# marja-w/gan-des-midi-music-gen

Hardware: AMD Instinct MI355X
Metric: GAN training samples/sec (G+D step) (higher is better)
Workload: dtype bf16; 1 GPU; SIMNN G/D iteration, synthetic 128x256 spectrogram windows; per_gpu_batch=256, global_batch=256, mode=faithful, parallelism=dp1

## Files before the change

gan_des_midi_music_gen_amd/csrc/adam_pc.h:

```cpp
#pragma once
#include "gdm_common.h"

__device__ __forceinline__ void adam_derived(const float* hyper, int step, float& step_size, float& bc2_sqrt) {
  const double b1 = (double)hyper[2], b2 = (double)hyper[3];
  step_size = (float)((double)hyper[1] / (1.0 - pow(b1, (double)step)));
  bc2_sqrt = (float)sqrt(1.0 - pow(b2, (double)step));
}

__device__ __forceinline__ void adam_pc_gather(float (&tile)[32][132], const float* __restrict__ g_pc, int C, int P,
                                               int bx, int by, int bz) {
  const int t = threadIdx.x, tx = t & 31, ty = t >> 5;
  const int p0 = bx * 128, c0 = by * 32;
  const int64_t base = (int64_t)bz * C * P;
#pragma unroll
  for (int i = 0; i < 16; ++i) {
    const int pl = ty + 8 * i, pp = p0 + pl, c = c0 + tx;
    tile[tx][pl] = (pp < P && c < C) ? g_pc[base + (int64_t)pp * C + c] : 0.f;
  }
}

template <typename TS>
__device__ __forceinline__ void adam_pc_update(float (&tile)[32][132], float* __restrict__ p, float* __restrict__ m,
                                               float* __restrict__ v, int C, int P, TS* __restrict__ shadow_pc,
                                               const float* __restrict__ hyper, int vec_ok, float step_size,
                                               float bc2_sqrt, int bx, int by, int bz) {
  const float w1 = 1.0f - hyper[2], beta2 = hyper[3], omb2 = 1.0f - hyper[3], eps = hyper[4], gscale = hyper[5];
  const int t = threadIdx.x, tx = t & 31, ty = t >> 5;
  const int p0 = bx * 128, c0 = by * 32, n = bz;
  const int64_t base = (int64_t)n * C * P;
  const bool full = vec_ok && p0 + 128 <= P && c0 + 32 <= C;
#pragma unroll
  for (int i = 0; i < 4; ++i) {
    const int cl = ty + 8 * i, c = c0 + cl, pp = p0 + 4 * tx;
    const int64_t k = base + (int64_t)c * P + pp;
    f32x4 gg = *(const f32x4*)&tile[cl][4 * tx], pv, mv, vv;
    if (full) {
#ifndef GDM_ADAM_DEFAULT_POLICY
      pv = __builtin_nontemporal_load((const f32x4*)(p + k)); mv = __builtin_nontemporal_load((const f32x4*)(m + k));
      vv = __builtin_nontemporal_load((const f32x4*)(v + k));
#else
      pv = *(const f32x4*)(p + k); mv = *(const f32x4*)(m + k); vv = *(const f32x4*)(v + k);
#endif
    } else {
#pragma unroll
      for (int e = 0; e < 4; ++e) {
        const bool ok = c < C && pp + e < P;
        pv[e] = ok ? p[k + e] : 0.f; mv[e] = ok ? m[k + e] : 0.f; vv[e] = ok ? v[k + e] : 0.f;
      }
    }
#pragma unroll
    for (int e = 0; e < 4; ++e) {
      float pj = pv[e], mj = mv[e], vj = vv[e];
      adam_element(pj, mj, vj, gg[e], gscale, w1, beta2, omb2, eps, step_size, bc2_sqrt);
      pv[e] = pj; mv[e] = mj; vv[e] = vj;
    }
    if (full) {
#ifndef GDM_ADAM_DEFAULT_POLICY
      __builtin_nontemporal_store(pv, (f32x4*)(p + k)); __builtin_nontemporal_store(mv, (f32x4*)(m + k));
      __builtin_nontemporal_store(vv, (f32x4*)(v + k));
#else
      *(f32x4*)(p + k) = pv; *(f32x4*)(m + k) = mv; *(f32x4*)(v + k) = vv;
#endif
    } else {
#pragma unroll
      for (int e = 0; e < 4; ++e)
        if (c < C && pp + e < P) { p[k + e] = pv[e]; m[k + e] = mv[e]; v[k + e] = vv[e]; }
    }
    *(f32x4*)&tile[cl][4 * tx] = pv;
  }
  __syncthreads();
#pragma unroll
  for (int i = 0; i < 16; ++i) {
    const int pl = ty + 8 * i, pp = p0 + pl, c = c0 + tx;
    if (pp < P && c < C) shadow_pc[base + (int64_t)pp * C + c] = from_f32<TS>(tile[tx][pl]);
  }
}


template <typename TS>
__device__ __forceinline__ void adam_pc_tile(float (&tile)[32][132], float* __restrict__ p, const float* __restrict__ g_pc,
                                             float* __restrict__ m, float* __restrict__ v, int C, int P,
                                             TS* __restrict__ shadow_pc, const float* __restrict__ hyper, int vec_ok,
                                             float step_size, float bc2_sqrt, int bx, int by, int bz) {
  adam_pc_gather(tile, g_pc, C, P, bx, by, bz);
  __syncthreads();
  adam_pc_update<TS>(tile, p, m, v, C, P, shadow_pc, hyper, vec_ok, step_size, bc2_sqrt, bx, by, bz);
}
```

gan_des_midi_music_gen_amd/csrc/pointwise.hip:

```cpp
#include "gdm_common.h"
#include "adam_pc.h"

namespace {

__global__ __launch_bounds__(1024) void bce_kernel(const float* __restrict__ x, float target, int n, float gscale,
                                                   float* __restrict__ loss, float* __restrict__ dx, int fuse_sig,
                                                   int accumulate) {
  __shared__ float red[1024];
  const int t = threadIdx.x;
  float s = 0.f;
  for (int i = t; i < n; i += 1024) {
    const float v = x[i];
    s += fmaxf(v, 0.f) - v * target + log1pf(expf(-fabsf(v)));
    if (dx) {
      float g = (1.0f / (1.0f + expf(-v)) - target) * gscale / (float)n;
      if (fuse_sig) g *= v * (1.f - v);
      dx[i] = g;
    }
  }
  red[t] = s;
  __syncthreads();
  for (int o = 512; o > 0; o >>= 1) {
    if (t < o) red[t] += red[t + o];
    __syncthreads();
// ... 85 lines not shown
        pp[j] = pj; mm[j] = mj; vv[j] = vj;
      }
      *(f32x4*)(p + i) = pp;
      *(f32x4*)(m + i) = mm;
      *(f32x4*)(v + i) = vv;
    } else {
      for (int64_t k = i; k < n && k < i + 4; ++k) {
        adam_element(p[k], m[k], v[k], g[k], gscale, w1, beta2, omb2, eps, step_size, bc2_sqrt);
      }
    }
  }
}

struct Welford { float n, mean, m2; };
__device__ __forceinline__ void welford_merge(Welford& a, const Welford& b) {
  if (b.n == 0.f) return;
  const float n = a.n + b.n;
  const float d = b.mean - a.mean;
  a.mean += d * (b.n / n);
  a.m2 += b.m2 + d * d * (a.n * b.n / n);
  a.n = n;
}

__device__ __forceinline__ Welford welford_from_shifted(float n, float shift, float s, float ss) {
  Welford a{n, 0.f, 0.f};
  if (n > 0.f) {
    a.mean = shift + s / n;
    a.m2 = fmaxf(ss - s * (s / n), 0.f);
  }
  return a;
}

__global__ __launch_bounds__(256) void bn_partial_stats(const float* __restrict__ y, int rows, int C, int chunk_rows,
                                                        int CW, float* __restrict__ ws) {
  __shared__ Welford sh[4][64];
  const int lane = threadIdx.x & 63, wv = threadIdx.x >> 6;
  const int rpl = 64 / CW;
  const int c = blockIdx.x * 64 + (lane & (CW - 1)), sub = lane / CW;
  const int r0 = blockIdx.y * chunk_rows, r1 = min(rows, r0 + chunk_rows);
  const int step = 4 * rpl;
  float n = 0.f, shift = 0.f, s = 0.f, ss = 0.f;
  if (c < C) {
    int r = r0 + wv * rpl + sub;
    if (r < r1) shift = y[(int64_t)r * C + c];
    for (; r + 7 * step < r1; r += 8 * step) {
      float x[8];
#pragma unroll
      for (int q = 0; q < 8; ++q) x[q] = y[(int64_t)(r + q * step) * C + c];
#pragma unroll
      for (int q = 0; q < 8; ++q) { const float d = x[q] - shift; s += d; ss += d * d; }
      n += 8.f;
    }
    for (; r < r1; r += step) { const float d = y[(int64_t)r * C + c] - shift; s += d; ss += d * d; n += 1.f; }
  }
  sh[wv][lane] = welford_from_shifted(n, shift, s, ss);
  __syncthreads();
  if (wv == 0 && sub == 0 && c < C) {
    Welford t{0.f, 0.f, 0.f};
    for (int w = 0; w < 4; ++w)
      for (int q = 0; q < rpl; ++q) welford_merge(t, sh[w][q * CW + lane]);
    float* o = ws + ((int64_t)blockIdx.y * C + c) * 3;
    o[0] = t.n; o[1] = t.mean; o[2] = t.m2;
  }
}

__global__ __launch_bounds__(1024) void bn_finalize(const float* __restrict__ ws, int chunks, int rows, int C,
                                                    float momentum, float eps, float* __restrict__ running_mean,
                                                    float* __restrict__ running_var, int64_t* __restrict__ nbt,
                                                    float* __restrict__ save_mean, float* __restrict__ save_invstd) {
  __shared__ Welford part[16][64];
  const int lane = threadIdx.x & 63, wv = threadIdx.x >> 6;
  const int c = blockIdx.x * 64 + lane;
  if (blockIdx.x == 0 && threadIdx.x == 0 && nbt) nbt[0] += 1;
  Welford t{0.f, 0.f, 0.f};
  if (c < C)
    for (int k = wv; k < chunks; k += 16 * 8) {
      Welford b[8];
#pragma unroll
      for (int q = 0; q < 8; ++q) {
        const int kk = k + 16 * q;
        const float* o = ws + ((int64_t)min(kk, chunks - 1) * C + c) * 3;
        b[q] = Welford{kk < chunks ? o[0] : 0.f, o[1], o[2]};
      }
#pragma unroll
      for (int q = 0; q < 8; ++q) welford_merge(t, b[q]);
    }
  part[wv][lane] = t;
  __syncthreads();
  if (wv != 0 || c >= C) return;
  t = part[0][lane];
#pragma unroll
  for (int w = 1; w < 16; ++w) welford_merge(t, part[w][lane]);
  const float var_b = t.m2 / (float)rows;
  save_mean[c] = t.mean;
  save_invstd[c] = 1.0f / sqrtf(var_b + eps);
  if (running_mean) {
    const float var_u = t.m2 / (float)max(rows - 1, 1);
    running_mean[c] = (1.f - momentum) * running_mean[c] + momentum * t.mean;
    running_var[c] = (1.f - momentum) * running_var[c] + momentum * var_u;
  }
}

__global__ __launch_bounds__(256) void bn_eval_stats(const float* __restrict__ running_mean,
                                                     const float* __restrict__ running_var, int C, float eps,
                                                     float* __restrict__ save_mean, float* __restrict__ save_invstd) {
  const int c = blockIdx.x * 256 + threadIdx.x;
  if (c >= C) return;
  save_mean[c] = running_mean[c];
  save_invstd[c] = 1.0f / sqrtf(running_var[c] + eps);
}

template <typename IT>
__global__ __launch_bounds__(256) void bn_apply(const float* __restrict__ y, int64_t total64, int C,
                                                const float* __restrict__ gamma, const float* __restrict__ beta,
                                                const float* __restrict__ mean, const float* __restrict__ invstd,
                                                int act, void* __restrict__ out, int out_dtype) {
  const IT total = (IT)total64, stride = (IT)gridDim.x * 256;
  for (IT i = (IT)blockIdx.x * 256 + threadIdx.x; i < total; i += stride) {
    const int c = (int)(i % C);
    const float alpha = invstd[c] * gamma[c];
    const float v = (y[i] - mean[c]) * alpha + beta[c];
    store_from_f32(out, out_dtype, i, apply_act(v, act, 0.f));
  }
}

__global__ __launch_bounds__(256) void bn_bwd_partial(const void* __restrict__ dout, const void* __restrict__ out,
                                                      int dtype, const float* __restrict__ y, int rows, int C,
                                                      int chunk_rows, const float* __restrict__ mean,
                                                      const float* __restrict__ invstd, int act,
                                                      float* __restrict__ ws) {
  __shared__ float sh1[4][64], sh2[4][64];
  const int lane = threadIdx.x & 63, wv = threadIdx.x >> 6;
  const int c = blockIdx.x * 64 + lane;
  const int r0 = blockIdx.y * chunk_rows, r1 = min(rows, r0 + chunk_rows);
  float s1 = 0.f, s2 = 0.f;
  if (c < C) {
    const float mu = mean[c], is = invstd[c];
    for (int r = r0 + wv; r < r1; r += 4) {
      const int64_t i = (int64_t)r * C + c;
      const float g = load_as_f32(dout, dtype, i) * act_grad_from_out(load_as_f32(out, dtype, i), act, 0.f);
      s1 += g;
      s2 += g * ((y[i] - mu) * is);
    }
  }
  sh1[wv][lane] = s1; sh2[wv][lane] = s2;
  __syncthreads();
  if (wv == 0 && c < C) {
    float* o = ws + ((int64_t)blockIdx.y * C + c) * 2;
    o[0] = ((sh1[0][lane] + sh1[1][lane]) + sh1[2][lane]) + sh1[3][lane];
    o[1] = ((sh2[0][lane] + sh2[1][lane]) + sh2[2][lane]) + sh2[3][lane];
  }
}

__global__ __launch_bounds__(256) void bn_bwd_finalize(const float* __restrict__ ws, int chunks, int C,
                                                       float* __restrict__ dgamma, float* __restrict__ dbeta) {
  const int c = blockIdx.x * 256 + threadIdx.x;
  if (c >= C) return;
  float s1 = 0.f, s2 = 0.f;
  for (int k = 0; k < chunks; ++k) {
    s1 += ws[((int64_t)k * C + c) * 2];
    s2 += ws[((int64_t)k * C + c) * 2 + 1];
  }
  dbeta[c] = s1;
  dgamma[c] = s2;
}

__global__ __launch_bounds__(256) void bn_bwd_apply(const void* __restrict__ dout, const void* __restrict__ out,
                                                    int dtype, const float* __restrict__ y, int64_t total, int rows,
                                                    int C, const float* __restrict__ gamma,
                                                    const float* __restrict__ mean, const float* __restrict__ invstd,
                                                    const float* __restrict__ dgamma, const float* __restrict__ dbeta,
                                                    int act, float* __restrict__ dy) {
  const int64_t stride = (int64_t)gridDim.x * 256;
  const float inv_r = 1.0f / (float)rows;
  for (int64_t i = (int64_t)blockIdx.x * 256 + threadIdx.x; i < total; i += stride) {
    const int c = (int)(i % C);
    const float g = load_as_f32(dout, dtype, i) * act_grad_from_out(load_as_f32(out, dtype, i), act, 0.f);
    const float xhat = (y[i] - mean[c]) * invstd[c];
    dy[i] = gamma[c] * invstd[c] * (g - dbeta[c] * inv_r - xhat * dgamma[c] * inv_r);
  }
}

__global__ __launch_bounds__(256) void bias_act_kernel(const float* __restrict__ x, const float* __restrict__ bias,
                                                       int64_t total, int cols, int act, float slope,
                                                       void* __restrict__ out, int out_dtype) {
  const int64_t stride = (int64_t)gridDim.x * 256;
  for (int64_t i = (int64_t)blockIdx.x * 256 + threadIdx.x; i < total; i += stride) {
    float v = x[i];
    if (bias) v += bias[i % cols];
    store_from_f32(out, out_dtype, i, apply_act(v, act, slope));
  }
}

__global__ __launch_bounds__(256) void act_bwd_kernel(const void* __restrict__ dout, const void* __restrict__ out,
                                                      int dtype, int64_t n, int act, float slope,
                                                      void* __restrict__ dx) {
  const int64_t stride = (int64_t)gridDim.x * 256;
  for (int64_t i = (int64_t)blockIdx.x * 256 + threadIdx.x; i < n; i += stride) {
    const float g = load_as_f32(dout, dtype, i) * act_grad_from_out(load_as_f32(out, dtype, i), act, slope);
    store_from_f32(dx, dtype, i, g);
  }
}

__global__ __launch_bounds__(256) void colsum_partial(const void* __restrict__ x, int dtype, int rows, int C,
                                                      int chunk_rows, float* __restrict__ ws) {
  __shared__ float sh[4][64];
  const int lane = threadIdx.x & 63, wv = threadIdx.x >> 6;
  const int c = blockIdx.x * 64 + lane;
  const int r0 = blockIdx.y * chunk_rows, r1 = min(rows, r0 + chunk_rows);
  float s = 0.f;
  if (c < C)
    for (int r = r0 + wv; r < r1; r += 4) s += load_as_f32(x, dtype, (int64_t)r * C + c);
  sh[wv][lane] = s;
  __syncthreads();
  if (wv == 0 && c < C) ws[(int64_t)blockIdx.y * C + c] = ((sh[0][lane] + sh[1][lane]) + sh[2][lane]) + sh[3][lane];
}

__global__ __launch_bounds__(256) void colsum_final(const float* __restrict__ ws, int chunks, int C,
                                                    float* __restrict__ out) {
  const int c = blockIdx.x * 256 + threadIdx.x;
  if (c >= C) return;
  float s = 0.f;
  for (int k = 0; k < chunks; ++k) s += ws[(int64_t)k * C + c];
  out[c] = s;
}

__global__ __launch_bounds__(256) void cast_kernel(const void* __restrict__ src, int sd, void* __restrict__ dst,
                                                   int dd, int64_t n) {
  const int64_t stride = (int64_t)gridDim.x * 256;
  for (int64_t i = (int64_t)blockIdx.x * 256 + threadIdx.x; i < n; i += stride)
    store_from_f32(dst, dd, i, load_as_f32(src, sd, i));
}

inline int row_chunks(int rows) {
  int c = (rows + 255) / 256;
  return c < 1 ? 1 : (c > 64 ? 64 : c);
}
inline unsigned grid_for(int64_t total) {
  int64_t b = (total + 255) / 256;
  return (unsigned)(b > 4096 ? 4096 : (b < 1 ? 1 : b));
}

}

extern "C" int gdm_bce_with_logits(const float* x, float target, int n, float grad_scale, float* loss, float* dx,
                                   int fuse_sigmoid_backward, int accumulate_loss, void* stream) {
  GDM_REQUIRE(x && loss, "gdm_bce_with_logits: null pointer");
  GDM_REQUIRE(n > 0 && n <= 65536, "gdm_bce_with_logits: n=%d out of range (1..65536)", n);
  hipLaunchKernelGGL(bce_kernel, dim3(1), dim3(1024), 0, (hipStream_t)stream, x, target, n, grad_scale, loss, dx,
                     fuse_sigmoid_backward, accumulate_loss);
  GDM_LAUNCH_OK("gdm_bce_with_logits");
  return GDM_OK;
}

extern "C" int gdm_criterion_loss(const float* x, float target, int n, int criterion, float grad_scale, float* loss,
                                  float* dx, int accumulate_loss, void* stream) {
  GDM_REQUIRE(x && loss, "gdm_criterion_loss: null pointer");
  GDM_REQUIRE(n > 0 && n <= 65536, "gdm_criterion_loss: n=%d out of range (1..65536)", n);
  GDM_REQUIRE(criterion == GDM_CRIT_BCE_LOGITS || criterion == GDM_CRIT_MSE || criterion == GDM_CRIT_L1,
              "gdm_criterion_loss: unknown criterion %d (GDM_CRIT_BCE_LOGITS, GDM_CRIT_MSE or GDM_CRIT_L1)", criterion);
  hipStream_t s = (hipStream_t)stream;
  if (criterion == GDM_CRIT_BCE_LOGITS)
    hipLaunchKernelGGL(bce_kernel, dim3(1), dim3(1024), 0, s, x, target, n, grad_scale, loss, dx, 0, accumulate_loss);
  else if (criterion == GDM_CRIT_MSE)
    hipLaunchKernelGGL(crit_kernel<GDM_CRIT_MSE>, dim3(1), dim3(1024), 0, s, x, target, n, grad_scale, loss, dx,
                       accumulate_loss);
  else
    hipLaunchKernelGGL(crit_kernel<GDM_CRIT_L1>, dim3(1), dim3(1024), 0, s, x, target, n, grad_scale, loss, dx,
                       accumulate_loss);
  GDM_LAUNCH_OK("gdm_criterion_loss");
  return GDM_OK;
}

extern "C" int gdm_adam_step(float* p, const float* g, float* m, float* v, int64_t n, int step, float lr, float beta1,
                             float beta2, float eps, float grad_scale, void* stream) {
  GDM_REQUIRE(p && g && m && v, "gdm_adam_step: null pointer");
  GDM_REQUIRE(n > 0 && step >= 1, "gdm_adam_step: bad n=%lld or step=%d", (long long)n, step);
  const bool aligned = (((uintptr_t)p | (uintptr_t)g | (uintptr_t)m | (uintptr_t)v) & 15) == 0;
  const double bc1 = 1.0 - pow((double)beta1, (double)step);
  const double bc2 = 1.0 - pow((double)beta2, (double)step);
  const float step_size = (float)((double)lr / bc1);
  const float bc2_sqrt = (float)sqrt(bc2);
  int64_t blocks = (n / 4 + 255) / 256;
  if (blocks < 1) blocks = 1;
  if (blocks > 8192) blocks = 8192;
  if (aligned)
    hipLaunchKernelGGL(adam_kernel<true>, dim3((unsigned)blocks), dim3(256), 0, (hipStream_t)stream, p, g, m, v, n,
                       1.0f - beta1, beta2, 1.0f - beta2, step_size, bc2_sqrt, eps, grad_scale);
  else
    hipLaunchKernelGGL(adam_kernel<false>, dim3((unsigned)blocks), dim3(256), 0, (hipStream_t)stream, p, g, m, v, n,
                       1.0f - beta1, beta2, 1.0f - beta2, step_size, bc2_sqrt, eps, grad_scale);
  GDM_LAUNCH_OK("gdm_adam_step");
  return GDM_OK;
}

extern "C" int gdm_adam_step_dev_pc(float* p, const float* g_pc, float* m, float* v, int N, int C, int P,
                                    void* shadow_pc, int shadow_dtype, float* hyper, int advance_step, void* stream) {
  GDM_REQUIRE(p && g_pc && m && v && shadow_pc && hyper, "gdm_adam_step_dev_pc: null pointer");
  GDM_REQUIRE(N > 0 && C > 0 && P > 0 && N <= 65535 && (C + 31) / 32 <= 65535 && gdm_dtype_ok(shadow_dtype),
              "gdm_adam_step_dev_pc: bad arguments");
  hipStream_t s = (hipStream_t)stream;
  if (advance_step) hipLaunchKernelGGL(adam_prep_kernel, dim3(1), dim3(1), 0, s, hyper);
  const dim3 grid((P + 127) / 128, (C + 31) / 32, N);
  const int vec_ok = (P % 4 == 0) && ((((uintptr_t)p | (uintptr_t)m | (uintptr_t)v) & 15) == 0);
  if (shadow_dtype == GDM_BF16)
    hipLaunchKernelGGL(adam_dev_pc_kernel<__bf16>, grid, dim3(256), 0, s, p, g_pc, m, v, C, P, (__bf16*)shadow_pc, hyper,
                       vec_ok);
  else
    hipLaunchKernelGGL(adam_dev_pc_kernel<float>, grid, dim3(256), 0, s, p, g_pc, m, v, C, P, (float*)shadow_pc, hyper,
                       vec_ok);
  GDM_LAUNCH_OK("gdm_adam_step_dev_pc");
  return GDM_OK;
}

extern "C" int gdm_adam_step_dev(float* p, const float* g, float* m, float* v, int64_t n, float* hyper, void* stream) {
  GDM_REQUIRE(p && g && m && v && hyper && n > 0, "gdm_adam_step_dev: bad arguments");
  const bool aligned = (((uintptr_t)p | (uintptr_t)g | (uintptr_t)m | (uintptr_t)v) & 15) == 0;
  int64_t blocks = (n / 4 + 255) / 256;
  if (blocks < 1) blocks = 1;
  if (blocks > 8192) blocks = 8192;
  hipStream_t s = (hipStream_t)stream;
  hipLaunchKernelGGL(adam_prep_kernel, dim3(1), dim3(1), 0, s, hyper);
  if (aligned) hipLaunchKernelGGL(adam_dev_kernel<true>, dim3((unsigned)blocks), dim3(256), 0, s, p, g, m, v, n, hyper);
  else hipLaunchKernelGGL(adam_dev_kernel<false>, dim3((unsigned)blocks), dim3(256), 0, s, p, g, m, v, n, hyper);
  GDM_LAUNCH_OK("gdm_adam_step_dev");
  return GDM_OK;
}

extern "C" size_t gdm_bn_workspace_bytes(int rows, int channels) {
  return (size_t)row_chunks(rows) * (size_t)channels * 3 * sizeof(float);
}

extern "C" int gdm_bn_act_fwd(const float* y, int rows, int channels, const float* gamma, const float* beta,
                              float* running_mean, float* running_var, int64_t* num_batches_tracked, float momentum,
                              float eps, int act, void* out, int out_dtype, float* save_mean, float* save_invstd,
                              int training, void* workspace, size_t workspace_bytes, void* stream) {
  GDM_REQUIRE(y && gamma && beta && out && save_mean && save_invstd, "gdm_bn_act_fwd: null pointer");
  GDM_REQUIRE(rows > 0 && channels > 0 && gdm_dtype_ok(out_dtype), "gdm_bn_act_fwd: bad arguments");
  hipStream_t s = (hipStream_t)stream;
  const int C = channels;
  if (training) {
    GDM_REQUIRE(rows > 1, "gdm_bn_act_fwd: training-mode batch norm needs more than 1 value per channel");
    const int chunks = row_chunks(rows);
    if (!workspace || workspace_bytes < gdm_bn_workspace_bytes(rows, C)) {
      gdm_set_error("gdm_bn_act_fwd: workspace too small");
      return GDM_EWORKSPACE;
    }
    const int chunk_rows = (rows + chunks - 1) / chunks;
    int cw = 64;
    while (cw / 2 >= C && cw > 1) cw /= 2;
    hipLaunchKernelGGL(bn_partial_stats, dim3((C + 63) / 64, chunks), dim3(256), 0, s, y, rows, C, chunk_rows, cw,
                       (float*)workspace);
    hipLaunchKernelGGL(bn_finalize, dim3((C + 63) / 64), dim3(1024), 0, s, (const float*)workspace, chunks, rows, C,
                       momentum, eps, running_mean, running_var, num_batches_tracked, save_mean, save_invstd);
  } else {
    GDM_REQUIRE(running_mean && running_var, "gdm_bn_act_fwd: eval mode needs running statistics");
    hipLaunchKernelGGL(bn_eval_stats, dim3((C + 255) / 256), dim3(256), 0, s, running_mean, running_var, C, eps,
                       save_mean, save_invstd);
  }
  const int64_t total = (int64_t)rows * C;
  if (total < ((int64_t)1 << 31))
    hipLaunchKernelGGL(bn_apply<int>, dim3(grid_for(total)), dim3(256), 0, s, y, total, C, gamma, beta, save_mean,
                       save_invstd, act, out, out_dtype);
  else
    hipLaunchKernelGGL(bn_apply<int64_t>, dim3(grid_for(total)), dim3(256), 0, s, y, total, C, gamma, beta, save_mean,
                       save_invstd, act, out, out_dtype);
  GDM_LAUNCH_OK("gdm_bn_act_fwd");
  return GDM_OK;
}

extern "C" int gdm_bn_partial_chunks(int rows) { return row_chunks(rows); }

extern "C" int gdm_bn_partials(const float* y, int rows, int channels, float* partials, void* stream) {
  GDM_REQUIRE(y && partials && rows > 0 && channels > 0, "gdm_bn_partials: bad arguments");
  const int C = channels, chunks = row_chunks(rows), chunk_rows = (rows + chunks - 1) / chunks;
  int cw = 64;
  while (cw / 2 >= C && cw > 1) cw /= 2;
  hipLaunchKernelGGL(bn_partial_stats, dim3((C + 63) / 64, chunks), dim3(256), 0, (hipStream_t)stream, y, rows, C,
                     chunk_rows, cw, partials);
  GDM_LAUNCH_OK("gdm_bn_partials");
  return GDM_OK;
}

extern "C" int gdm_bn_apply(const float* y, int rows, int channels, const float* gamma, const float* beta,
                            const float* mean, const float* invstd, int act, void* out, int out_dtype, void* stream) {
  GDM_REQUIRE(y && gamma && beta && mean && invstd && out && rows > 0 && channels > 0 && gdm_dtype_ok(out_dtype),
              "gdm_bn_apply: bad arguments");
  const int64_t total = (int64_t)rows * channels;
  hipStream_t s = (hipStream_t)stream;
  if (total < ((int64_t)1 << 31))
    hipLaunchKernelGGL(bn_apply<int>, dim3(grid_for(total)), dim3(256), 0, s, y, total, channels, gamma, beta, mean, invstd,
                       act, out, out_dtype);
  else
    hipLaunchKernelGGL(bn_apply<int64_t>, dim3(grid_for(total)), dim3(256), 0, s, y, total, channels, gamma, beta, mean,
                       invstd, act, out, out_dtype);
  GDM_LAUNCH_OK("gdm_bn_apply");
  return GDM_OK;
}

extern "C" int gdm_bn_finalize(const float* ws, int chunks, int rows, int channels, float momentum, float eps,
                               float* running_mean, float* running_var, int64_t* num_batches_tracked, float* save_mean,
                               float* save_invstd, void* stream) {
  GDM_REQUIRE(ws && save_mean && save_invstd && chunks > 0 && rows > 1 && channels > 0, "gdm_bn_finalize: bad arguments");
  hipLaunchKernelGGL(bn_finalize, dim3((channels + 63) / 64), dim3(1024), 0, (hipStream_t)stream, ws, chunks, rows,
                     channels, momentum, eps, running_mean, running_var, num_batches_tracked, save_mean, save_invstd);
  GDM_LAUNCH_OK("gdm_bn_finalize");
  return GDM_OK;
}

extern "C" int gdm_bn_stats(const float* y, int rows, int channels, float* running_mean, float* running_var,
                            int64_t* num_batches_tracked, float momentum, float eps, float* save_mean,
                            float* save_invstd, void* workspace, size_t workspace_bytes, void* stream) {
  GDM_REQUIRE(y && save_mean && save_invstd && rows > 1 && channels > 0, "gdm_bn_stats: bad arguments");
  if (!workspace || workspace_bytes < gdm_bn_workspace_bytes(rows, channels)) {
    gdm_set_error("gdm_bn_stats: workspace too small");
    return GDM_EWORKSPACE;
  }
  hipStream_t s = (hipStream_t)stream;
  const int C = channels, chunks = row_chunks(rows), chunk_rows = (rows + chunks - 1) / chunks;
  int cw = 64;
  while (cw / 2 >= C && cw > 1) cw /= 2;
  hipLaunchKernelGGL(bn_partial_stats, dim3((C + 63) / 64, chunks), dim3(256), 0, s, y, rows, C, chunk_rows, cw,
                     (float*)workspace);
  hipLaunchKernelGGL(bn_finalize, dim3((C + 63) / 64), dim3(1024), 0, s, (const float*)workspace, chunks, rows, C,
                     momentum, eps, running_mean, running_var, num_batches_tracked, save_mean, save_invstd);
  GDM_LAUNCH_OK("gdm_bn_stats");
  return GDM_OK;
}

extern "C" int gdm_bn_act_bwd(const void* dout, const void* out, int out_dtype, const float* y, int rows, int channels,
                              const float* gamma, const float* save_mean, const float* save_invstd, int act,
                              float* dy, float* dgamma, float* dbeta, void* workspace, size_t workspace_bytes,
                              void* stream) {
  GDM_REQUIRE(dout && out && y && gamma && save_mean && save_invstd && dy && dgamma && dbeta,
              "gdm_bn_act_bwd: null pointer");
  GDM_REQUIRE(rows > 0 && channels > 0 && gdm_dtype_ok(out_dtype), "gdm_bn_act_bwd: bad arguments");
  const int C = channels, chunks = row_chunks(rows);
  if (!workspace || workspace_bytes < gdm_bn_workspace_bytes(rows, C)) {
    gdm_set_error("gdm_bn_act_bwd: workspace too small");
    return GDM_EWORKSPACE;
  }
  hipStream_t s = (hipStream_t)stream;
  const int chunk_rows = (rows + chunks - 1) / chunks;
  hipLaunchKernelGGL(bn_bwd_partial, dim3((C + 63) / 64, chunks), dim3(256), 0, s, dout, out, out_dtype, y, rows, C,
                     chunk_rows, save_mean, save_invstd, act, (float*)workspace);
  hipLaunchKernelGGL(bn_bwd_finalize, dim3((C + 255) / 256), dim3(256), 0, s, (const float*)workspace, chunks, C,
                     dgamma, dbeta);
  const int64_t total = (int64_t)rows * C;
  hipLaunchKernelGGL(bn_bwd_apply, dim3(grid_for(total)), dim3(256), 0, s, dout, out, out_dtype, y, total, rows, C,
                     gamma, save_mean, save_invstd, dgamma, dbeta, act, dy);
  GDM_LAUNCH_OK("gdm_bn_act_bwd");
  return GDM_OK;
}

extern "C" int gdm_bias_act_fwd(const float* x, const float* bias, int rows, int cols, int act, float slope, void* out,
                                int out_dtype, void* stream) {
  GDM_REQUIRE(x && out && rows > 0 && cols > 0 && gdm_dtype_ok(out_dtype), "gdm_bias_act_fwd: bad arguments");
  const int64_t total = (int64_t)rows * cols;
  hipLaunchKernelGGL(bias_act_kernel, dim3(grid_for(total)), dim3(256), 0, (hipStream_t)stream, x, bias, total, cols,
                     act, slope, out, out_dtype);
  GDM_LAUNCH_OK("gdm_bias_act_fwd");
  return GDM_OK;
}

extern "C" int gdm_act_bwd(const void* dout, const void* out, int dtype, int64_t n, int act, float slope, void* dx,
                           void* stream) {
  GDM_REQUIRE(dout && out && dx && n > 0 && gdm_dtype_ok(dtype), "gdm_act_bwd: bad arguments");
  hipLaunchKernelGGL(act_bwd_kernel, dim3(grid_for(n)), dim3(256), 0, (hipStream_t)stream, dout, out, dtype, n, act,
                     slope, dx);
  GDM_LAUNCH_OK("gdm_act_bwd");
  return GDM_OK;
}

extern "C" int gdm_colsum(const void* x, int dtype, int rows, int cols, float* out, void* workspace,
                          size_t workspace_bytes, void* stream) {
  GDM_REQUIRE(x && out && rows > 0 && cols > 0 && gdm_dtype_ok(dtype), "gdm_colsum: bad arguments");
  const int chunks = row_chunks(rows);
  if (!workspace || workspace_bytes < (size_t)chunks * cols * sizeof(float)) {
    gdm_set_error("gdm_colsum: workspace too small (need %zu)", (size_t)chunks * cols * sizeof(float));
    return GDM_EWORKSPACE;
  }
  hipStream_t s = (hipStream_t)stream;
  const int chunk_rows = (rows + chunks - 1) / chunks;
  hipLaunchKernelGGL(colsum_partial, dim3((cols + 63) / 64, chunks), dim3(256), 0, s, x, dtype, rows, cols, chunk_rows,
                     (float*)workspace);
  hipLaunchKernelGGL(colsum_final, dim3((cols + 255) / 256), dim3(256), 0, s, (const float*)workspace, chunks, cols,
                     out);
  GDM_LAUNCH_OK("gdm_colsum");
  return GDM_OK;
}

extern "C" int gdm_cast(const void* src, int src_dtype, void* dst, int dst_dtype, int64_t n, void* stream) {
  GDM_REQUIRE(src && dst && n > 0 && gdm_dtype_ok(src_dtype) && gdm_dtype_ok(dst_dtype), "gdm_cast: bad arguments");
  hipLaunchKernelGGL(cast_kernel, dim3(grid_for(n)), dim3(256), 0, (hipStream_t)stream, src, src_dtype, dst,
                     dst_dtype, n);
  GDM_LAUNCH_OK("gdm_cast");
  return GDM_OK;
}

namespace {
constexpr int HEAD_ROWS = 8;
__global__ __launch_bounds__(256) void simnn_head_kernel(const float* __restrict__ h1, const float* __restrict__ w2,
                                                         const float* __restrict__ b2, int n, int n0, float y0,
                                                         float y1, float* __restrict__ prob, void* __restrict__ dh1,
                                                         int dh1_bf16, float* __restrict__ partials) {
  __shared__ float dz_s[HEAD_ROWS], lt_s[HEAD_ROWS], part[2][256];
  const int t = threadIdx.x, lane = t & 63, wv = t >> 6;
  const int r0 = blockIdx.x * HEAD_ROWS, r1 = min(n, r0 + HEAD_ROWS);
  const float wa = w2[lane], wb = w2[lane + 64], bias = b2[0];
  float hv[HEAD_ROWS / 4][2];
#pragma unroll
  for (int k = 0; k < HEAD_ROWS / 4; ++k) {
    const int b = r0 + wv + 4 * k;
    hv[k][0] = b < r1 ? h1[(int64_t)b * 128 + lane] : 0.f;
    hv[k][1] = b < r1 ? h1[(int64_t)b * 128 + 64 + lane] : 0.f;
  }
#pragma unroll
  for (int k = 0; k < HEAD_ROWS / 4; ++k) {
    const int b = r0 + wv + 4 * k, bl = wv + 4 * k;
    const float s = wave_sum(hv[k][0] * wa + hv[k][1] * wb);
    if (lane == 0) {
      float lt = 0.f, dz = 0.f;
      if (b < r1) {
        const float z = s + bias;
        const float p = 1.0f / (1.0f + expf(-z));
        const bool first = b < n0;
        const float y = first ? y0 : y1;
        const float cnt = (float)(first ? n0 : n - n0);
        prob[b] = p;
        lt = (fmaxf(p, 0.f) - p * y + log1pf(expf(-fabsf(p)))) / cnt;
        dz = (1.0f / (1.0f + expf(-p)) - y) / cnt * p * (1.f - p);
      }
      lt_s[bl] = lt;
      dz_s[bl] = dz;
    }
  }
  __syncthreads();
  float* po = partials + (int64_t)blockIdx.x * 258;
  if (t == 0) {
    float l = 0.f, sdz = 0.f;
#pragma unroll
    for (int b = 0; b < HEAD_ROWS; ++b) { l += lt_s[b]; sdz += dz_s[b]; }
    po[256] = sdz;
    po[257] = l;
  }
  const int j = t & 127, grp = t >> 7;
  const float wj = w2[j];
  float s_w = 0.f, s_b1 = 0.f;
  float hh[HEAD_ROWS / 2];
#pragma unroll
  for (int k = 0; k < HEAD_ROWS / 2; ++k) {
    const int b = r0 + grp + 2 * k;
    hh[k] = b < r1 ? h1[(int64_t)b * 128 + j] : 0.f;
  }
#pragma unroll
  for (int k = 0; k < HEAD_ROWS / 2; ++k) {
    const int b = r0 + grp + 2 * k;
    const float d = dz_s[grp + 2 * k];
    const float g = hh[k] > 0.f ? d * wj : 0.f;
    if (dh1 != nullptr && b < r1) {
      if (dh1_bf16) ((__bf16*)dh1)[(int64_t)b * 128 + j] = (__bf16)g;
      else ((float*)dh1)[(int64_t)b * 128 + j] = g;
    }
    s_w = fmaf(d, hh[k], s_w);
    s_b1 += g;
  }
  part[0][t] = s_w;
  part[1][t] = s_b1;
  __syncthreads();
  if (t < 128) {
    po[t] = part[0][t] + part[0][128 + t];
    po[128 + t] = part[1][t] + part[1][128 + t];
  }
}

__global__ __launch_bounds__(320) void simnn_head_final(const float* __restrict__ partials, int groups,
                                                        float* __restrict__ loss, int accumulate_loss,
                                                        float* __restrict__ dw2, float* __restrict__ db2,
                                                        float* __restrict__ db1) {
  const int t = threadIdx.x;
  if (t >= 258) return;
  float p8[8] = {0.f, 0.f, 0.f, 0.f, 0.f, 0.f, 0.f, 0.f};
  int g = 0;
  for (; g + 8 <= groups; g += 8) {
#pragma unroll
    for (int q = 0; q < 8; ++q) p8[q] += partials[(int64_t)(g + q) * 258 + t];
  }
  for (; g < groups; ++g) p8[0] += partials[(int64_t)g * 258 + t];
  const float s = ((p8[0] + p8[1]) + (p8[2] + p8[3])) + ((p8[4] + p8[5]) + (p8[6] + p8[7]));
  if (t == 257) loss[0] = (accumulate_loss ? loss[0] : 0.f) + s;
  else if (dw2 != nullptr) {
    if (t < 128) dw2[t] = s;
    else if (t < 256) db1[t - 128] = s;
    else db2[0] = s;
  }
}
}

extern "C" size_t gdm_simnn_head_workspace_bytes(int n) {
  return (size_t)((n + HEAD_ROWS - 1) / HEAD_ROWS) * 258 * sizeof(float);
}

extern "C" int gdm_simnn_head(const float* h1, const float* w2, const float* b2, int n, int n0, float y0, float y1,
                              float* prob, float* loss, int accumulate_loss, void* dh1, int dh1_dtype, float* dw2,
                              float* db2, float* db1, void* workspace, size_t workspace_bytes, void* stream) {
  GDM_REQUIRE(h1 && w2 && b2 && prob && loss, "gdm_simnn_head: null pointer");
  GDM_REQUIRE(n > 0 && n <= 65536 && n0 > 0 && n0 <= n, "gdm_simnn_head: bad batch n=%d n0=%d", n, n0);
// ... 72 lines not shown
```

gan_des_midi_music_gen_amd/csrc/simnn_adam.hip:

```cpp
#include "simnn_trunk.h"
#include "adam_pc.h"

namespace {

constexpr int REC_SLOT0 = 16, REC_GROUP0 = 32, REC_GROUPS = 64;
constexpr int REC_INTS = REC_GROUP0 + 16 * REC_GROUPS;
template <typename T>
__global__ __launch_bounds__(256, 8) void simnn_adam_kernel(float* __restrict__ p, const float* __restrict__ g_pc,
                                                         float* __restrict__ m, float* __restrict__ v, int C, int P,
                                                         T* __restrict__ shadow_pc, int vec_ok, int tiles_x, int tiles_y,
                                                         int small_vec_ok, float* __restrict__ ps,
                                                         const float* __restrict__ gs, float* __restrict__ ms,
                                                         float* __restrict__ vs, int n_small,
                                                         const float* __restrict__ w2, T* __restrict__ wf,
                                                         T* __restrict__ wb, float* __restrict__ hyper, int* rec) {
  __shared__ __attribute__((aligned(16))) float lds[4608];
  static_assert(sizeof(lds) >= sizeof(float[32][132]), "tile");
  float (&tile)[32][132] = *reinterpret_cast<float (*)[32][132]>(lds);
  __shared__ float hy[2];
  STAMP_DECL;
  const int step = __float_as_int(hyper[0]) + 1;
  const int tag0 = rec[REC_SLOT0], tag1 = rec[REC_SLOT0 + 4];
  const float ss0 = __int_as_float(rec[REC_SLOT0 + 1]), bq0 = __int_as_float(rec[REC_SLOT0 + 2]);
  const float ss1 = __int_as_float(rec[REC_SLOT0 + 5]), bq1 = __int_as_float(rec[REC_SLOT0 + 6]);
  float step_size, bc2_sqrt;
  auto resolve = [&]() {
    const bool odd = step & 1;
    step_size = odd ? ss1 : ss0;
    bc2_sqrt = odd ? bq1 : bq0;
    if ((odd ? tag1 : tag0) != step) {
      if (threadIdx.x == 0) adam_derived(hyper, step, hy[0], hy[1]);
      __syncthreads();
      step_size = hy[0]; bc2_sqrt = hy[1];
    }
  };
  const int blk = blockIdx.x;
  STAMP(0);
  if (blk == 0) {
    resolve();
    const float w1 = 1.0f - hyper[2], beta2 = hyper[3], omb2 = 1.0f - hyper[3], eps = hyper[4], gscale = hyper[5];
    const int w2_off = (int)(w2 - ps);
    auto keep_w2 = [&](int i, float val) {
      const unsigned j = (unsigned)(i - w2_off);
      if (j < 4608u) lds[j] = val;
    };
    const int n4 = small_vec_ok ? n_small / 4 : 0;
    constexpr int R = 2;
    for (int v0 = threadIdx.x; v0 < n4; v0 += 256 * R) {
      f32x4 pj[R], mj[R], vj[R], gj[R];
#pragma unroll
      for (int r = 0; r < R; ++r) {
        const int iv = min(v0 + 256 * r, n4 - 1);
        pj[r] = ((const f32x4*)ps)[iv]; mj[r] = ((const f32x4*)ms)[iv]; vj[r] = ((const f32x4*)vs)[iv];
        gj[r] = ((const f32x4*)gs)[iv];
      }
#pragma unroll
      for (int r = 0; r < R; ++r) {
        const int iv = v0 + 256 * r;
#pragma unroll
        for (int e = 0; e < 4; ++e) {
          float a = pj[r][e], bm = mj[r][e], bv = vj[r][e];
          adam_element(a, bm, bv, gj[r][e], gscale, w1, beta2, omb2, eps, step_size, bc2_sqrt);
          pj[r][e] = a; mj[r][e] = bm; vj[r][e] = bv;
          if (iv < n4) keep_w2(4 * iv + e, a);
        }
        if (iv < n4) { ((f32x4*)ps)[iv] = pj[r]; ((f32x4*)ms)[iv] = mj[r]; ((f32x4*)vs)[iv] = vj[r]; }
      }
    }
    for (int i = 4 * n4 + threadIdx.x; i < n_small; i += 256) {
      float a = ps[i], bm = ms[i], bv = vs[i];
      adam_element(a, bm, bv, gs[i], gscale, w1, beta2, omb2, eps, step_size, bc2_sqrt);
      ps[i] = a; ms[i] = bm; vs[i] = bv;
      keep_w2(i, a);
    }
    __syncthreads();
    STAMP(1);
    constexpr int U = 4;
    for (int i0 = threadIdx.x; i0 < C2<T>::WF_ELEMS; i0 += 256 * U) {
      float val[U];
#pragma unroll
      for (int u = 0; u < U; ++u) {
        val[u] = conv2_packed_value<T, false>(lds, min(i0 + 256 * u, C2<T>::WF_ELEMS - 1));
      }
#pragma unroll
      for (int u = 0; u < U; ++u)
        if (i0 + 256 * u < C2<T>::WF_ELEMS) wf[i0 + 256 * u] = from_f32<T>(val[u]);
    }
    for (int i0 = threadIdx.x; i0 < C2<T>::WB_ELEMS; i0 += 256 * U) {
      float val[U];
#pragma unroll
      for (int u = 0; u < U; ++u) {
        val[u] = conv2_packed_value<T, true>(lds, min(i0 + 256 * u, C2<T>::WB_ELEMS - 1));
      }
#pragma unroll
      for (int u = 0; u < U; ++u)
        if (i0 + 256 * u < C2<T>::WB_ELEMS) wb[i0 + 256 * u] = from_f32<T>(val[u]);
    }
    STAMP(2);
    if (threadIdx.x == 255) {
      float ss, bq;
      adam_derived(hyper, step + 1, ss, bq);
      int* nxt = rec + REC_SLOT0 + 4 * ((step + 1) & 1);
      nxt[1] = __float_as_int(ss); nxt[2] = __float_as_int(bq); nxt[0] = step + 1;
    }
    __syncthreads();
    STAMP(3);
  }
  {
    const int bx = blk % tiles_x, by = (blk / tiles_x) % tiles_y, bz = blk / (tiles_x * tiles_y);
    adam_pc_gather(tile, g_pc, C, P, bx, by, bz);
    resolve();
    __syncthreads();
    adam_pc_update<T>(tile, p, m, v, C, P, shadow_pc, hyper, vec_ok, step_size, bc2_sqrt, bx, by, bz);
  }
  __syncthreads();
  STAMP(4);
  STAMP_FLUSH;
  if (threadIdx.x == 0) {
    const int grp = (int)blockIdx.x % REC_GROUPS, n_grp = min((int)gridDim.x, REC_GROUPS);
    const int in_grp = ((int)gridDim.x - grp + REC_GROUPS - 1) / REC_GROUPS;
    if (atomicAdd(rec + REC_GROUP0 + 16 * grp, 1) == in_grp - 1) {
      atomicExch(rec + REC_GROUP0 + 16 * grp, 0);
      if (atomicAdd(rec, 1) == n_grp - 1) {
        atomicExch(rec, 0);
        hyper[0] = __int_as_float(step);
        hyper[6] = step_size;
        hyper[7] = bc2_sqrt;
      }
    }
  }
}

}

extern "C" int gdm_simnn_adam_step(float* p_big, const float* g_big_pc, float* m_big, float* v_big, int N, int C, int P,
                                   void* shadow_pc, float* p_small, const float* g_small, float* m_small, float* v_small,
                                   int n_small, const float* conv2_weight, void* pack, int dtype, float* hyper, int* done,
                                   void* stream) {
  GDM_REQUIRE(p_big && g_big_pc && m_big && v_big && shadow_pc && p_small && g_small && m_small && v_small && conv2_weight &&
              pack && hyper && done, "gdm_simnn_adam_step: null pointer");
  GDM_REQUIRE(N > 0 && C > 0 && P > 0 && n_small > 0 && gdm_dtype_ok(dtype), "gdm_simnn_adam_step: bad arguments");
  GDM_REQUIRE(conv2_weight >= p_small && conv2_weight + 4608 <= p_small + n_small,
              "gdm_simnn_adam_step: conv2.weight must lie inside the small-parameter range (it is re-packed from there)");
  const int tx = (P + 127) / 128, ty = (C + 31) / 32;
  const int64_t nbig = (int64_t)tx * ty * N;
  GDM_REQUIRE(nbig < ((int64_t)1 << 30), "gdm_simnn_adam_step: parameter too large");
  const int vec_ok = (P % 4 == 0) && ((((uintptr_t)p_big | (uintptr_t)m_big | (uintptr_t)v_big) & 15) == 0);
  const int small_vec_ok = ((((uintptr_t)p_small | (uintptr_t)g_small | (uintptr_t)m_small | (uintptr_t)v_small) & 15) == 0);
  DISPATCH_T(dtype, hipLaunchKernelGGL(simnn_adam_kernel<T>, dim3((unsigned)nbig), dim3(256), 0, (hipStream_t)stream, p_big,
                                       g_big_pc, m_big, v_big, C, P, (T*)shadow_pc, vec_ok, tx, ty, small_vec_ok, p_small, g_small,
                                       m_small, v_small, n_small, conv2_weight, (T*)pack, (T*)pack + C2<T>::WF_ELEMS, hyper,
                                       done));
  static_assert(REC_INTS == GDM_SIMNN_ADAM_RECORD_INTS, "include/gdm.h states the record's size");
  GDM_LAUNCH_OK("gdm_simnn_adam_step");
  return GDM_OK;
}

GDM_STAMP_READER(adam)
```

Measured before the change: 418,400 samples/s.

## Vectorize and prefetch Adam per-channel tile loads with swizzled LDS transpose

Reworks the per-channel Adam tile update so that when C==32 the gradient gather and the shadow-copy scatter use 16-byte contiguous vector accesses instead of scalar strided ones. The tile index is XOR-swizzled to avoid LDS bank conflicts. The first row of p/m/v is loaded early, overlapping the gather and the resolve barrier, and later rows are software-prefetched. This is meant to cut memory-instruction count and latency in the optimizer step, at the cost of more registers and a more complex indexing scheme.

```diff
diff --git a/gan_des_midi_music_gen_amd/csrc/adam_pc.h b/gan_des_midi_music_gen_amd/csrc/adam_pc.h
--- a/gan_des_midi_music_gen_amd/csrc/adam_pc.h
+++ b/gan_des_midi_music_gen_amd/csrc/adam_pc.h
@@ -7,72 +7,155 @@
   bc2_sqrt = (float)sqrt(1.0 - pow(b2, (double)step));
 }
 
-__device__ __forceinline__ void adam_pc_gather(float (&tile)[32][132], const float* __restrict__ g_pc, int C, int P,
-                                               int bx, int by, int bz) {
+constexpr int ADAM_PC_VEC = 1, ADAM_PC_WIDE = 2;
+
+static inline int adam_pc_flags(const float* p, const float* m, const float* v, const float* g_pc,
+                                const void* shadow_pc, int C, int P) {
+  const int vec = (P % 4 == 0) && ((((uintptr_t)p | (uintptr_t)m | (uintptr_t)v) & 15) == 0);
+  const int wide = C == 32 && ((((uintptr_t)g_pc | (uintptr_t)shadow_pc) & 15) == 0);
+  return (vec ? ADAM_PC_VEC : 0) | (wide ? ADAM_PC_WIDE : 0);
+}
+
+__device__ __forceinline__ f32x4 adam_pc_load4(const float* a) {
+#ifndef GDM_ADAM_DEFAULT_POLICY
+  return __builtin_nontemporal_load((const f32x4*)a);
+#else
+  return *(const f32x4*)a;
+#endif
+}
+__device__ __forceinline__ f32x4 adam_pc_load_g4(const float* a) {
+#ifndef GDM_ADAM_G_DEFAULT_POLICY
+  return __builtin_nontemporal_load((const f32x4*)a);
+#else
+  return *(const f32x4*)a;
+#endif
+}
+__device__ __forceinline__ void adam_pc_store4(f32x4 x, float* a) {
+#ifndef GDM_ADAM_DEFAULT_POLICY
+  __builtin_nontemporal_store(x, (f32x4*)a);
+#else
+  *(f32x4*)a = x;
+#endif
+}
+
+struct AdamPcEarly { f32x4 p, m, v; };
+
+__device__ __forceinline__ void adam_pc_gather(float (&tile)[32][132], const float* __restrict__ g_pc,
+                                               const float* __restrict__ p, const float* __restrict__ m,
+                                               const float* __restrict__ v, int C, int P, int flags, int bx, int by,
+                                               int bz, AdamPcEarly& early) {
   const int t = threadIdx.x, tx = t & 31, ty = t >> 5;
   const int p0 = bx * 128, c0 = by * 32;
   const int64_t base = (int64_t)bz * C * P;
+  const bool full = (flags & ADAM_PC_VEC) && p0 + 128 <= P && c0 + 32 <= C;
+  const int64_t k0 = base + (int64_t)(c0 + ty) * P + p0 + 4 * tx;
+  if ((flags & ADAM_PC_WIDE) && p0 + 128 <= P) {
+    const float* src = g_pc + base + (int64_t)p0 * 32 + 4 * t;
+    f32x4 g[4];
+#pragma unroll
+    for (int j = 0; j < 4; ++j) g[j] = adam_pc_load_g4(src + 1024 * j);
+    if (full) { early.p = adam_pc_load4(p + k0); early.m = adam_pc_load4(m + k0); early.v = adam_pc_load4(v + k0); }
+    const int c4 = 4 * (t & 7);
+#pragma unroll
+    for (int j = 0; j < 4; ++j) {
+      const int col = ((t >> 3) + 32 * j) ^ c4;
+#pragma unroll
+      for (int e = 0; e < 4; ++e) tile[c4 + e][col] = g[j][e];
+    }
+    return;
+  }
+  float g[16];
 #pragma unroll
   for (int i = 0; i < 16; ++i) {
-    const int pl = ty + 8 * i, pp = p0 + pl, c = c0 + tx;
-    tile[tx][pl] = (pp < P && c < C) ? g_pc[base + (int64_t)pp * C + c] : 0.f;
+    const int pp = p0 + ty + 8 * i, c = c0 + tx;
+    g[i] = (pp < P && c < C) ? g_pc[base + (int64_t)pp * C + c] : 0.f;
   }
+  if (full) { early.p = adam_pc_load4(p + k0); early.m = adam_pc_load4(m + k0); early.v = adam_pc_load4(v + k0); }
+#pragma unroll
+  for (int i = 0; i < 16; ++i) tile[tx][(ty + 8 * i) ^ (tx & 28)] = g[i];
 }
 
 template <typename TS>
 __device__ __forceinline__ void adam_pc_update(float (&tile)[32][132], float* __restrict__ p, float* __restrict__ m,
                                                float* __restrict__ v, int C, int P, TS* __restrict__ shadow_pc,
-                                               const float* __restrict__ hyper, int vec_ok, float step_size,
-                                               float bc2_sqrt, int bx, int by, int bz) {
+                                               const float* __restrict__ hyper, int flags, float step_size,
+                                               float bc2_sqrt, int bx, int by, int bz, const AdamPcEarly& early) {
   const float w1 = 1.0f - hyper[2], beta2 = hyper[3], omb2 = 1.0f - hyper[3], eps = hyper[4], gscale = hyper[5];
   const int t = threadIdx.x, tx = t & 31, ty = t >> 5;
   const int p0 = bx * 128, c0 = by * 32, n = bz;
   const int64_t base = (int64_t)n * C * P;
-  const bool full = vec_ok && p0 + 128 <= P && c0 + 32 <= C;
+  const bool full = (flags & ADAM_PC_VEC) && p0 + 128 <= P && c0 + 32 <= C;
+  if (full) {
+    f32x4 pv = early.p, mv = early.m, vv = early.v;
 #pragma unroll
-  for (int i = 0; i < 4; ++i) {
-    const int cl = ty + 8 * i, c = c0 + cl, pp = p0 + 4 * tx;
-    const int64_t k = base + (int64_t)c * P + pp;
-    f32x4 gg = *(const f32x4*)&tile[cl][4 * tx], pv, mv, vv;
-    if (full) {
-#ifndef GDM_ADAM_DEFAULT_POLICY
-      pv = __builtin_nontemporal_load((const f32x4*)(p + k)); mv = __builtin_nontemporal_load((const f32x4*)(m + k));
-      vv = __builtin_nontemporal_load((const f32x4*)(v + k));
-#else
-      pv = *(const f32x4*)(p + k); mv = *(const f32x4*)(m + k); vv = *(const f32x4*)(v + k);
-#endif
-    } else {
+    for (int i = 0; i < 4; ++i) {
+      const int cl = ty + 8 * i;
+      const int64_t k = base + (int64_t)(c0 + cl) * P + p0 + 4 * tx;
+      f32x4 pn, mn, vn;
+      if (i < 3) {
+        const int64_t kn = k + (int64_t)8 * P;
+        pn = adam_pc_load4(p + kn); mn = adam_pc_load4(m + kn); vn = adam_pc_load4(v + kn);
+      }
+      float* trow = &tile[cl][(4 * tx) ^ (cl & 28)];
+      const f32x4 gg = *(const f32x4*)trow;
+#pragma unroll
+      for (int e = 0; e < 4; ++e) {
+        float pj = pv[e], mj = mv[e], vj = vv[e];
+        adam_element(pj, mj, vj, gg[e], gscale, w1, beta2, omb2, eps, step_size, bc2_sqrt);
+        pv[e] = pj; mv[e] = mj; vv[e] = vj;
+      }
+      adam_pc_store4(pv, p + k); adam_pc_store4(mv, m + k); adam_pc_store4(vv, v + k);
+      *(f32x4*)trow = pv;
+      if (i < 3) { pv = pn; mv = mn; vv = vn; }
+    }
+  } else {
+#pragma unroll
+    for (int i = 0; i < 4; ++i) {
+      const int cl = ty + 8 * i, c = c0 + cl, pp = p0 + 4 * tx;
+      const int64_t k = base + (int64_t)c * P + pp;
+      float* trow = &tile[cl][(4 * tx) ^ (cl & 28)];
+      f32x4 gg = *(const f32x4*)trow, pv, mv, vv;
 #pragma unroll
       for (int e = 0; e < 4; ++e) {
         const bool ok = c < C && pp + e < P;
         pv[e] = ok ? p[k + e] : 0.f; mv[e] = ok ? m[k + e] : 0.f; vv[e] = ok ? v[k + e] : 0.f;
       }
-    }
 #pragma unroll
-    for (int e = 0; e < 4; ++e) {
-      float pj = pv[e], mj = mv[e], vj = vv[e];
-      adam_element(pj, mj, vj, gg[e], gscale, w1, beta2, omb2, eps, step_size, bc2_sqrt);
-      pv[e] = pj; mv[e] = mj; vv[e] = vj;
-    }
-    if (full) {
-#ifndef GDM_ADAM_DEFAULT_POLICY
-      __builtin_nontemporal_store(pv, (f32x4*)(p + k)); __builtin_nontemporal_store(mv, (f32x4*)(m + k));
-      __builtin_nontemporal_store(vv, (f32x4*)(v + k));
-#else
-      *(f32x4*)(p + k) = pv; *(f32x4*)(m + k) = mv; *(f32x4*)(v + k) = vv;
-#endif
-    } else {
+      for (int e = 0; e < 4; ++e) {
+        float pj = pv[e], mj = mv[e], vj = vv[e];
+        adam_element(pj, mj, vj, gg[e], gscale, w1, beta2, omb2, eps, step_size, bc2_sqrt);
+        pv[e] = pj; mv[e] = mj; vv[e] = vj;
+      }
 #pragma unroll
       for (int e = 0; e < 4; ++e)
         if (c < C && pp + e < P) { p[k + e] = pv[e]; m[k + e] = mv[e]; v[k + e] = vv[e]; }
+      *(f32x4*)trow = pv;
     }
-    *(f32x4*)&tile[cl][4 * tx] = pv;
   }
   __syncthreads();
+  if ((flags & ADAM_PC_WIDE) && p0 + 128 <= P) {
+    constexpr int E = 16 / (int)sizeof(TS), CG = 32 / E;
+    typedef TS ts_vec __attribute__((ext_vector_type(E)));
+    ts_vec* dst = (ts_vec*)(shadow_pc + base + (int64_t)p0 * 32) + t;
+    const int ce = E * (t % CG);
+#pragma unroll
+    for (int j = 0; j < 16 / E; ++j) {
+      const int pl = t / CG + (256 / CG) * j;
+      ts_vec o;
+#pragma unroll
+      for (int e = 0; e < E; ++e) o[e] = from_f32<TS>(tile[ce + e][pl ^ ((ce + e) & 28)]);
+#ifndef GDM_ADAM_COPY_NONTEMPORAL
+      dst[256 * j] = o;
+#else
+      __builtin_nontemporal_store(o, dst + 256 * j);
+#endif
+    }
+    return;
+  }
 #pragma unroll
   for (int i = 0; i < 16; ++i) {
     const int pl = ty + 8 * i, pp = p0 + pl, c = c0 + tx;
-    if (pp < P && c < C) shadow_pc[base + (int64_t)pp * C + c] = from_f32<TS>(tile[tx][pl]);
+    if (pp < P && c < C) shadow_pc[base + (int64_t)pp * C + c] = from_f32<TS>(tile[tx][pl ^ (tx & 28)]);
   }
 }
 
@@ -80,9 +163,10 @@
 template <typename TS>
 __device__ __forceinline__ void adam_pc_tile(float (&tile)[32][132], float* __restrict__ p, const float* __restrict__ g_pc,
                                              float* __restrict__ m, float* __restrict__ v, int C, int P,
-                                             TS* __restrict__ shadow_pc, const float* __restrict__ hyper, int vec_ok,
+                                             TS* __restrict__ shadow_pc, const float* __restrict__ hyper, int flags,
                                              float step_size, float bc2_sqrt, int bx, int by, int bz) {
-  adam_pc_gather(tile, g_pc, C, P, bx, by, bz);
+  AdamPcEarly early;
+  adam_pc_gather(tile, g_pc, p, m, v, C, P, flags, bx, by, bz, early);
   __syncthreads();
-  adam_pc_update<TS>(tile, p, m, v, C, P, shadow_pc, hyper, vec_ok, step_size, bc2_sqrt, bx, by, bz);
+  adam_pc_update<TS>(tile, p, m, v, C, P, shadow_pc, hyper, flags, step_size, bc2_sqrt, bx, by, bz, early);
 }
diff --git a/gan_des_midi_music_gen_amd/csrc/pointwise.hip b/gan_des_midi_music_gen_amd/csrc/pointwise.hip
--- a/gan_des_midi_music_gen_amd/csrc/pointwise.hip
+++ b/gan_des_midi_music_gen_amd/csrc/pointwise.hip
@@ -411,7 +411,7 @@
   hipStream_t s = (hipStream_t)stream;
   if (advance_step) hipLaunchKernelGGL(adam_prep_kernel, dim3(1), dim3(1), 0, s, hyper);
   const dim3 grid((P + 127) / 128, (C + 31) / 32, N);
-  const int vec_ok = (P % 4 == 0) && ((((uintptr_t)p | (uintptr_t)m | (uintptr_t)v) & 15) == 0);
+  const int vec_ok = adam_pc_flags(p, m, v, g_pc, shadow_pc, C, P);
   if (shadow_dtype == GDM_BF16)
     hipLaunchKernelGGL(adam_dev_pc_kernel<__bf16>, grid, dim3(256), 0, s, p, g_pc, m, v, C, P, (__bf16*)shadow_pc, hyper,
                        vec_ok);
diff --git a/gan_des_midi_music_gen_amd/csrc/simnn_adam.hip b/gan_des_midi_music_gen_amd/csrc/simnn_adam.hip
--- a/gan_des_midi_music_gen_amd/csrc/simnn_adam.hip
+++ b/gan_des_midi_music_gen_amd/csrc/simnn_adam.hip
@@ -108,10 +108,11 @@
   }
   {
     const int bx = blk % tiles_x, by = (blk / tiles_x) % tiles_y, bz = blk / (tiles_x * tiles_y);
-    adam_pc_gather(tile, g_pc, C, P, bx, by, bz);
+    AdamPcEarly early;
+    adam_pc_gather(tile, g_pc, p, m, v, C, P, vec_ok, bx, by, bz, early);
     resolve();
     __syncthreads();
-    adam_pc_update<T>(tile, p, m, v, C, P, shadow_pc, hyper, vec_ok, step_size, bc2_sqrt, bx, by, bz);
+    adam_pc_update<T>(tile, p, m, v, C, P, shadow_pc, hyper, vec_ok, step_size, bc2_sqrt, bx, by, bz, early);
   }
   __syncthreads();
   STAMP(4);
@@ -145,7 +146,7 @@
   const int tx = (P + 127) / 128, ty = (C + 31) / 32;
   const int64_t nbig = (int64_t)tx * ty * N;
   GDM_REQUIRE(nbig < ((int64_t)1 << 30), "gdm_simnn_adam_step: parameter too large");
-  const int vec_ok = (P % 4 == 0) && ((((uintptr_t)p_big | (uintptr_t)m_big | (uintptr_t)v_big) & 15) == 0);
+  const int vec_ok = adam_pc_flags(p_big, m_big, v_big, g_big_pc, shadow_pc, C, P);
   const int small_vec_ok = ((((uintptr_t)p_small | (uintptr_t)g_small | (uintptr_t)m_small | (uintptr_t)v_small) & 15) == 0);
   DISPATCH_T(dtype, hipLaunchKernelGGL(simnn_adam_kernel<T>, dim3((unsigned)nbig), dim3(256), 0, (hipStream_t)stream, p_big,
                                        g_big_pc, m_big, v_big, C, P, (T*)shadow_pc, vec_ok, tx, ty, small_vec_ok, p_small, g_small,
```

Result: faster. 428,600 samples/s, median of 6 (+2.4%).
